# jianzhnie/ScaleRL

Measured on AMD Instinct MI355X. Metric: env_steps_per_sec, higher is better.
Workload: dtype bf16; 1 GPU; model=IMPALA AtariNet (3conv+FC512+2xLSTM519), algo=impala-vtrace, rollout_length=80, global_batch=256, seq_len=80, envs_per_actor=256, actors_per_rank=24, inference=gpu, parallelism=dp1

## Files before the change

scalerl_amd/ops/_backend.py:

```python

from __future__ import annotations

import ctypes
import os
import subprocess
import sys
from typing import Optional

import torch

_THIS_DIR = os.path.dirname(os.path.abspath(__file__))
_CSRC = os.path.join(_THIS_DIR, "csrc")
_SO_PATH = os.path.join(_THIS_DIR, "_hip_ops.so")

_LIB: Optional[ctypes.CDLL] = None
_LOAD_ERROR: Optional[str] = None


def hip_sources():
    return sorted(
        os.path.join(_CSRC, f) for f in os.listdir(_CSRC) if f.endswith(".hip"))


def build(verbose: bool = True, arch: str = "gfx950") -> str:
    srcs = hip_sources()
    hdrs = sorted(
        os.path.join(_CSRC, f) for f in os.listdir(_CSRC) if f.endswith(".h"))
    if os.path.exists(_SO_PATH):
        newest = max(os.path.getmtime(p) for p in srcs + hdrs)
        if os.path.getmtime(_SO_PATH) >= newest:
            return _SO_PATH
    hipcc = os.environ.get("HIPCC", "hipcc")
    cmd = [hipcc, f"--offload-arch={arch}", "-O3", "-std=c++17", "-shared",
           "-fPIC", "-lrocblas", "-o", _SO_PATH] + srcs
    if verbose:
        print("[scalerl_amd.ops] building:", " ".join(cmd), file=sys.stderr)
    subprocess.run(cmd, check=True)
    return _SO_PATH


_CONV_FWD = "bf16 bf16 f32? bf16 long int"
_CONV1_FWD_U8 = "u8 bf16 f32? bf16 long int"
_CONV_WGRAD = "bf16 bf16 f32 long long"
_CONV_WGRAD_V3 = "bf16 bf16 f32 long"
_CONV_DGRAD = "bf16 bf16 bf16 long"
_SIGNATURES = {
    "impala_fused_loss": "f32 f32 i64 f32 f32 f32 f32 float float float float"
                         " float long long long f32 f32 f32 f32?",
    "vtrace_from_log_rhos": "f32 f32 f32 f32 f32 float float float long long"
                            " f32 f32",
    "gae_scan": "f32 f32 f32 f32 float long long f32 f32",
    "discounted_returns": "f32 f32 f32? long long f32",
    "nstep_fold": "f32 f32 float long long long f32 f32 i32",
    "fused_rmsprop": "f32 f32 f32 f32? long float float float float float",
    "fused_adam": "f32 f32 f32 f32 long float float float float float long",
    "fused_polyak": "f32 f32 long float",
    "grad_clip_by_norm": "f32 long f32 float",
    "fused_td_loss": "f32 f32? f32 i64 f32 f32 f32? f32? f32? float long long"
                     " long int float long float float f32 f32 f32",
    "ppo_fused_loss": "f32 i64 f32 f32 f32 f32 float float float long long"
                      " f32 f32 f32",
    "per_update": "f32 long i64 f32 long",
    "per_sample": "f32 long long f32 long i64 f32",
    "per_leaf_min": "f32 long long i32",
    "lstm_mask_rows": "f32 f32 f32 f32 f32 long long",
    "lstm_cell_fwd": "f32 f32 f32 f32 f32? f32? f32? long long",
    "lstm_cell_bwd": "f32 f32 f32 f32 f32 f32? f32 f32 f32 long long",
    "masked_lstm_seq_fwd": "f32 f32 f32 f32 f32 f32 f32 f32 f32 long long long",
    "masked_lstm_seq_bwd": "f32 f32 f32 f32 f32 f32 f32 f32 f32 f32 long long"
                           " long",
    "frame_cast_u8_bf16": "u8 bf16 long",
    "mfma_selftest": "f32 f32 f32",
    "atari_encoder_fwd": "u8 bf16 f32 bf16 f32 bf16 f32 bf16? bf16? bf16 long",
    "atari_conv1_fwd_u8": _CONV1_FWD_U8,
    "atari_conv1_fwd_bf16": _CONV_FWD,
    "atari_conv2_fwd": _CONV_FWD,
    "atari_conv3_fwd": _CONV_FWD,
    "atari_conv2_fwd_v3": _CONV_FWD,
    "atari_conv3_fwd_v3": _CONV_FWD,
    "atari_conv1_wgrad_u8": "u8 bf16 f32 long long",
    "atari_conv2_wgrad": _CONV_WGRAD,
    "atari_conv3_wgrad": _CONV_WGRAD,
    "atari_conv1_wgrad_v3": "u8 bf16 f32 long",
    "atari_conv2_wgrad_v3": _CONV_WGRAD_V3,
    "atari_conv3_wgrad_v3": _CONV_WGRAD_V3,
    "atari_conv2_dgrad": _CONV_DGRAD,
    "atari_conv3_dgrad": _CONV_DGRAD,
    "atari_conv2_dgrad_v3": _CONV_DGRAD,
}

_DTYPES = {"f32": torch.float32, "i64": torch.int64, "i32": torch.int32,
           "bf16": torch.bfloat16, "u8": torch.uint8}
_SCALARS = {"long": ctypes.c_long, "int": ctypes.c_int,
            "float": ctypes.c_float}


class _Spec:
    __slots__ = ("words", "dtypes", "nullable", "argtypes", "fn")

    def __init__(self, words):
        self.words = words
        self.dtypes = tuple(_DTYPES.get(w.rstrip("?")) for w in words)
        self.nullable = tuple(w.endswith("?") for w in words)
        self.argtypes = [_SCALARS.get(w, ctypes.c_void_p) for w in words]
        self.argtypes.append(ctypes.c_void_p)
        self.fn = None


_SPECS = {name: _Spec(sig.split()) for name, sig in _SIGNATURES.items()}


def lib() -> ctypes.CDLL:
    global _LIB, _LOAD_ERROR
    if _LIB is not None:
        return _LIB
    if not os.path.exists(_SO_PATH):
        raise RuntimeError(
            f"scalerl_amd HIP kernel library not found at {_SO_PATH}. "
            f"Build it with `python -c 'from scalerl_amd.ops import _backend; "
            f"_backend.build()'` or `python setup.py build_ext --inplace`. "
            f"GPU execution without the native kernels is not supported.")
    try:
        loaded = ctypes.CDLL(_SO_PATH)
    except OSError as e:
        _LOAD_ERROR = str(e)
        raise RuntimeError(f"failed to load {_SO_PATH}: {e}") from e
    for name, spec in _SPECS.items():
        fn = getattr(loaded, name)
        fn.argtypes = spec.argtypes
        fn.restype = ctypes.c_int
        spec.fn = fn
    _LIB = loaded
    return _LIB


def available() -> bool:
    return os.path.exists(_SO_PATH)


def _reject(name: str, spec: _Spec, args) -> None:
    if len(args) != len(spec.words):
        raise TypeError(f"HIP kernel {name} takes {len(spec.words)} arguments "
                        f"({' '.join(spec.words)}), got {len(args)}")
    tensors = []
    for i, (a, dtype, nullable, word) in enumerate(
            zip(args, spec.dtypes, spec.nullable, spec.words)):
        where = f"HIP kernel {name}, argument {i} ({word})"
        if a is None:
            if nullable:
                continue
            raise TypeError(f"{where}: None given, the kernel takes " +
                            ("a number" if dtype is None
                             else "no null pointer") + " here")
        if dtype is None:
            continue
        if not isinstance(a, torch.Tensor):
            raise TypeError(f"{where}: expected a {dtype} tensor, got "
                            f"{type(a).__name__}")
        if a.dtype != dtype:
            raise TypeError(f"{where}: expected dtype {dtype}, got {a.dtype}")
        if not a.is_contiguous():
            raise ValueError(f"{where}: expected a contiguous tensor, got "
                             f"shape {tuple(a.shape)} stride {a.stride()}")
        tensors.append((where, a))
    for where, a in tensors:
        if not a.is_cuda:
            raise ValueError(f"{where}: expected a tensor on the current GPU, "
                             f"got device {a.device}")
    cur = torch.cuda.current_device()
    for where, a in tensors:
        if a.device.index != cur:
            raise ValueError(f"{where}: tensor is on {a.device} but the "
                             f"current device, whose stream the kernel is "
                             f"enqueued on, is cuda:{cur}")
    raise AssertionError(f"HIP kernel {name}: launch rejected valid arguments")


def launch(name: str, *args) -> None:
    spec = _SPECS.get(name)
    if spec is None:
        raise ValueError(f"unknown HIP kernel {name!r}")
    if len(args) != len(spec.words):
        _reject(name, spec, args)
    try:
        cur = torch.cuda.current_device()
    except (RuntimeError, AssertionError):
        cur = -2
    raw = []
    add = raw.append
    try:
        for a, dtype in zip(args, spec.dtypes):
            if dtype is None or a is None:
                add(a)
            elif (a.dtype is dtype and a.is_contiguous()
                  and a.get_device() == cur):
                add(a.data_ptr())
            else:
                _reject(name, spec, args)
    except AttributeError:
        _reject(name, spec, args)
    if None in raw and any(a is None and not ok
                           for a, ok in zip(args, spec.nullable)):
        _reject(name, spec, args)
    fn = spec.fn
    if fn is None:
        lib()
        fn = spec.fn
    ret = fn(*raw, torch._C._cuda_getCurrentRawStream(cur))
    if ret != 0:
        hint = ""
        if ret == -2:
            hint = " (action-space size exceeds kernel MAX_A)"
        elif ret == -3:
            hint = " (rollout length exceeds LDS budget)"
        elif ret == -4:
            hint = " (atom count outside the C51 kernel's 2..1024)"
        raise RuntimeError(
            f"HIP kernel {name} failed with code {ret}{hint}; "
            f"device={torch.cuda.get_device_name()}")
```

scalerl_amd/ops/csrc/lstm.hip:

```cpp

#include "lstm_cell.h"

extern "C" __global__ void lstm_mask_rows_kernel(
    const float* a, const float* b,
    const float* __restrict__ notdone,
    float* a_out, float* b_out, long B, long H) {
  const long total = B * H;
  for (long i = (long)blockIdx.x * blockDim.x + threadIdx.x; i < total;
       i += (long)gridDim.x * blockDim.x) {
    const float nd = notdone[i / H];
    a_out[i] = a[i] * nd;
    if (b != nullptr) b_out[i] = b[i] * nd;
  }
}

extern "C" __global__ void lstm_cell_fwd_kernel(
    float* __restrict__ gates,
    const float* __restrict__ c_in,
    float* __restrict__ h_out,
    float* __restrict__ c_out,
    const float* __restrict__ nd_next,
    float* __restrict__ h_in_next,
    float* __restrict__ c_in_next,
    long B, long H) {
  const long total = B * H;
  for (long i = (long)blockIdx.x * blockDim.x + threadIdx.x; i < total;
       i += (long)gridDim.x * blockDim.x) {
    const long b = i / H, j = i % H;
    float* grow = gates + b * 4 * H;
    const float ig = sigmoidf_(grow[j]);
    const float fg = sigmoidf_(grow[H + j]);
    const float gg = tanhf(grow[2 * H + j]);
    const float og = sigmoidf_(grow[3 * H + j]);
    const float c = fg * c_in[i] + ig * gg;
    const float h = og * tanhf(c);
    grow[j] = ig;
    grow[H + j] = fg;
    grow[2 * H + j] = gg;
    grow[3 * H + j] = og;
    c_out[i] = c;
    h_out[i] = h;
    if (nd_next != nullptr) {
      const float nd = nd_next[b];
      h_in_next[i] = h * nd;
      c_in_next[i] = c * nd;
    }
  }
}

extern "C" __global__ void lstm_cell_bwd_kernel(
    const float* __restrict__ gates,
    const float* __restrict__ c_in,
    const float* __restrict__ c_out,
    const float* __restrict__ d_hs_t,
    const float* __restrict__ g,
    const float* __restrict__ nd_next,
    const float* __restrict__ nd_t,
    float* dc_carry,
    float* __restrict__ dgates,
    long B, long H) {
  const long total = B * H;
  for (long i = (long)blockIdx.x * blockDim.x + threadIdx.x; i < total;
       i += (long)gridDim.x * blockDim.x) {
    const long b = i / H, j = i % H;
    const float* grow = gates + b * 4 * H;
    float* dgrow = dgates + b * 4 * H;
    const float ig = grow[j];
    const float fg = grow[H + j];
    const float gg = grow[2 * H + j];
    const float og = grow[3 * H + j];
    const float tc = tanhf(c_out[i]);
    const float gm = (nd_next != nullptr) ? g[i] * nd_next[b] : g[i];
    const float dh = d_hs_t[i] + gm;
    float tc2;
    {
#pragma clang fp contract(off)
      tc2 = tc * tc;
    }
    const float dc = dc_carry[i] + dh * og * (1.f - tc2);
    dgrow[j] = dc * gg * ig * (1.f - ig);
    dgrow[H + j] = dc * c_in[i] * fg * (1.f - fg);
    dgrow[2 * H + j] = dc * ig * (1.f - gg * gg);
    dgrow[3 * H + j] = dh * tc * og * (1.f - og);
    dc_carry[i] = (dc * fg) * nd_t[b];
  }
}

void lstm_launch_mask_rows(const float* a, const float* b, const float* notdone,
                           float* a_out, float* b_out, long B, long H,
                           hipStream_t stream) {
  hipLaunchKernelGGL(lstm_mask_rows_kernel,
                     dim3(grid_1d(B * H, LSTM_CELL_BLOCK)),
                     dim3(LSTM_CELL_BLOCK), 0, stream, a, b, notdone, a_out,
                     b_out, B, H);
}

void lstm_launch_cell_fwd(float* gates, const float* c_in, float* h_out,
                          float* c_out, const float* nd_next, float* h_in_next,
                          float* c_in_next, long B, long H,
                          hipStream_t stream) {
  hipLaunchKernelGGL(lstm_cell_fwd_kernel,
                     dim3(grid_1d(B * H, LSTM_CELL_BLOCK)),
                     dim3(LSTM_CELL_BLOCK), 0, stream, gates, c_in, h_out,
                     c_out, nd_next, h_in_next, c_in_next, B, H);
}

void lstm_launch_cell_bwd(const float* gates, const float* c_in,
                          const float* c_out, const float* d_hs_t,
                          const float* g, const float* nd_next,
                          const float* nd_t, float* dc_carry, float* dgates,
                          long B, long H, hipStream_t stream) {
  hipLaunchKernelGGL(lstm_cell_bwd_kernel,
                     dim3(grid_1d(B * H, LSTM_CELL_BLOCK)),
                     dim3(LSTM_CELL_BLOCK), 0, stream, gates, c_in, c_out,
                     d_hs_t, g, nd_next, nd_t, dc_carry, dgates, B, H);
}

extern "C" int lstm_mask_rows(const float* a, const float* b,
                              const float* notdone, float* a_out,
                              float* b_out, long B, long H,
                              hipStream_t stream) {
  if (B <= 0 || H <= 0) return 0;
  lstm_launch_mask_rows(a, b, notdone, a_out, b_out, B, H, stream);
  CHECK_LAUNCH();
  return 0;
}

extern "C" int lstm_cell_fwd(float* gates, const float* c_in, float* h_out,
                             float* c_out, const float* nd_next,
                             float* h_in_next, float* c_in_next, long B,
                             long H, hipStream_t stream) {
  if (B <= 0 || H <= 0) return 0;
  lstm_launch_cell_fwd(gates, c_in, h_out, c_out, nd_next, h_in_next,
                       c_in_next, B, H, stream);
  CHECK_LAUNCH();
  return 0;
}

extern "C" int lstm_cell_bwd(const float* gates, const float* c_in,
                             const float* c_out, const float* d_hs_t,
                             const float* g, const float* nd_next,
                             const float* nd_t, float* dc_carry,
                             float* dgates, long B, long H,
                             hipStream_t stream) {
  if (B <= 0 || H <= 0) return 0;
  lstm_launch_cell_bwd(gates, c_in, c_out, d_hs_t, g, nd_next, nd_t,
                       dc_carry, dgates, B, H, stream);
  CHECK_LAUNCH();
  return 0;
}
```

scalerl_amd/ops/csrc/lstm_cell.h:

```cpp
#pragma once

#include "common.h"

#define LSTM_CELL_BLOCK 256

void lstm_launch_mask_rows(const float* a, const float* b, const float* notdone,
                           float* a_out, float* b_out, long B, long H,
                           hipStream_t stream);

void lstm_launch_cell_fwd(float* gates, const float* c_in, float* h_out,
                          float* c_out, const float* nd_next, float* h_in_next,
                          float* c_in_next, long B, long H, hipStream_t stream);

void lstm_launch_cell_bwd(const float* gates, const float* c_in,
                          const float* c_out, const float* d_hs_t,
                          const float* g, const float* nd_next,
                          const float* nd_t, float* dc_carry, float* dgates,
                          long B, long H, hipStream_t stream);
```

scalerl_amd/ops/lstm.py:

```python

from __future__ import annotations

from typing import List, Tuple

import torch
import torch.nn as nn

from ._backend import launch


def _pointwise_fwd(gates: torch.Tensor, c_prev: torch.Tensor,
                   out_h: torch.Tensor = None, out_c: torch.Tensor = None):
    i, f, g, o = gates.chunk(4, dim=1)
    i, f, g, o = i.sigmoid(), f.sigmoid(), g.tanh(), o.sigmoid()
    c_new = f * c_prev + i * g
    h_new = o * torch.tanh(c_new)
    gates.copy_(torch.cat([i, f, g, o], dim=1))
    if out_h is not None:
        out_h.copy_(h_new)
        h_new = out_h
    if out_c is not None:
        out_c.copy_(c_new)
        c_new = out_c
    return h_new, c_new


def _pointwise_bwd(gates_act, c_prev, c_out, dh, dc_in,
                   out_dgates: torch.Tensor = None,
                   out_dc_prev: torch.Tensor = None):
    i, f, g, o = gates_act.chunk(4, dim=1)
    tc = torch.tanh(c_out)
    dc = dh * o * (1 - tc * tc)
    if dc_in is not None:
        dc = dc + dc_in
    di = dc * g * i * (1 - i)
    df = dc * c_prev * f * (1 - f)
    dg = dc * i * (1 - g * g)
    do = dh * tc * o * (1 - o)
    dgates = torch.cat([di, df, dg, do], dim=1)
    dc_prev = dc * f
    if out_dgates is not None:
        out_dgates.copy_(dgates)
        dgates = out_dgates
    if out_dc_prev is not None:
        out_dc_prev.copy_(dc_prev)
        dc_prev = out_dc_prev
    return dgates, dc_prev


def _grad_epilogue(dgates_all, x, hs_in, w_ih):
    T, B, I = x.shape
    dg2 = dgates_all.reshape(T * B, dgates_all.shape[-1])
    dx = (dg2 @ w_ih).view(T, B, I)
    dw_ih = dg2.t() @ x.reshape(T * B, I)
    dw_hh = dg2.t() @ hs_in.reshape(T * B, hs_in.shape[-1])
    db = dg2.sum(0)
    return dx, dw_ih, dw_hh, db


class _MaskedLSTMFn(torch.autograd.Function):

    @staticmethod
    @torch.amp.custom_fwd(device_type="cuda", cast_inputs=torch.float32)
    def forward(ctx, x, notdone, h0, c0, w_ih, w_hh, b_ih, b_hh):
        T, B, I = x.shape
        H = w_hh.shape[1]
        xg = torch.addmm(b_ih + b_hh, x.reshape(T * B, I), w_ih.t()).view(T, B, 4 * H)
        hs = torch.empty(T, B, H, device=x.device, dtype=x.dtype)
        cs_in = torch.empty(T, B, H, device=x.device, dtype=x.dtype)
        cs_out = torch.empty(T, B, H, device=x.device, dtype=x.dtype)
        hs_in = torch.empty(T, B, H, device=x.device, dtype=x.dtype)
        w_hh_t = w_hh.t()
        ctx.H = H
        if x.is_cuda:
            nd = notdone.reshape(T, B).contiguous()
            launch("lstm_mask_rows", h0.contiguous(), c0.contiguous(), nd[0],
                   hs_in[0], cs_in[0], B, H)
            for t in range(T):
                xg[t].addmm_(hs_in[t], w_hh_t)
                last = t == T - 1
                launch("lstm_cell_fwd",
                       xg[t], cs_in[t], hs[t], cs_out[t],
                       None if last else nd[t + 1],
                       None if last else hs_in[t + 1],
                       None if last else cs_in[t + 1], B, H)
            ctx.save_for_backward(x, nd, hs_in, cs_in, cs_out, xg, w_ih,
                                  w_hh)
            return hs, hs[T - 1].clone(), cs_out[T - 1].clone()
        h, c = h0.contiguous(), c0.contiguous()
        gates_all = torch.empty(T, B, 4 * H, device=x.device, dtype=x.dtype)
        for t in range(T):
            nd = notdone[t]
            h = torch.mul(h, nd, out=hs_in[t])
            c = torch.mul(c, nd, out=cs_in[t])
            torch.addmm(xg[t], h, w_hh_t, out=gates_all[t])
            h, c = _pointwise_fwd(gates_all[t], c, out_h=hs[t],
                                  out_c=cs_out[t])
        ctx.save_for_backward(x, notdone, hs_in, cs_in, cs_out, gates_all,
                              w_ih, w_hh)
        return hs, h.clone(), c.clone()

    @staticmethod
    @torch.amp.custom_bwd(device_type="cuda")
    def backward(ctx, d_hs, d_hT, d_cT):
        (x, notdone, hs_in, cs_in, cs_out, gates_all, w_ih,
         w_hh) = ctx.saved_tensors
        T, B, I = x.shape
        dgates_all = torch.empty_like(gates_all)
        if x.is_cuda:
            H = ctx.H
            nd = notdone
            d_hs_c = d_hs.contiguous()
            d_hT_c = d_hT.contiguous()
            dc_carry = d_cT.contiguous().clone()
            g = torch.empty_like(dc_carry)
            for t in range(T - 1, -1, -1):
                last = t == T - 1
                launch("lstm_cell_bwd",
                       gates_all[t], cs_in[t], cs_out[t],
                       d_hs_c[t], d_hT_c if last else g,
                       None if last else nd[t + 1], nd[t],
                       dc_carry, dgates_all[t], B, H)
                torch.mm(dgates_all[t], w_hh, out=g)
            dh0 = g.mul_(nd[0].unsqueeze(1))
            dx, dw_ih, dw_hh, db = _grad_epilogue(dgates_all, x, hs_in, w_ih)
            return dx, None, dh0, dc_carry, dw_ih, dw_hh, db, db
        dh_carry = d_hT.contiguous().clone()
        dc_carry = d_cT.contiguous().clone()
        dh_buf = torch.empty_like(dh_carry)
        dc_prev_buf = torch.empty_like(dc_carry)
        for t in range(T - 1, -1, -1):
            dh = torch.add(d_hs[t], dh_carry, out=dh_buf)
            dgates, dc_prev = _pointwise_bwd(
                gates_all[t], cs_in[t], cs_out[t], dh, dc_carry,
                out_dgates=dgates_all[t], out_dc_prev=dc_prev_buf)
            nd = notdone[t]
            torch.mm(dgates, w_hh, out=dh_carry)
            dh_carry.mul_(nd)
            torch.mul(dc_prev, nd, out=dc_carry)
        dx, dw_ih, dw_hh, db = _grad_epilogue(dgates_all, x, hs_in, w_ih)
        return dx, None, dh_carry, dc_carry, dw_ih, dw_hh, db, db


class _MaskedLSTMSeqFn(torch.autograd.Function):

    @staticmethod
    @torch.amp.custom_fwd(device_type="cuda", cast_inputs=torch.float32)
    def forward(ctx, x, notdone, h0, c0, w_ih, w_hh, b_ih, b_hh):
        T, B, I = x.shape
        H = w_hh.shape[1]
        dev = x.device
        xg = torch.addmm(b_ih + b_hh, x.reshape(T * B, I),
                         w_ih.t()).view(T, B, 4 * H).contiguous()
        hs = torch.empty(T, B, H, device=dev)
        hs_in = torch.empty(T, B, H, device=dev)
        cs_in = torch.empty(T, B, H, device=dev)
        cs_out = torch.empty(T, B, H, device=dev)
        nd = notdone.reshape(T, B).contiguous()
        w_hh_c = w_hh.contiguous()
        launch("masked_lstm_seq_fwd", xg, w_hh_c, nd, h0.contiguous(),
               c0.contiguous(), hs, hs_in, cs_in, cs_out, T, B, H)
        ctx.save_for_backward(x, nd, hs_in, cs_in, cs_out, xg, w_ih, w_hh_c)
        ctx.H = H
        return hs, hs[T - 1].clone(), cs_out[T - 1].clone()

    @staticmethod
    @torch.amp.custom_bwd(device_type="cuda")
    def backward(ctx, d_hs, d_hT, d_cT):
        x, nd, hs_in, cs_in, cs_out, gates_all, w_ih, w_hh = ctx.saved_tensors
        T, B, I = x.shape
        H = ctx.H
        dev = x.device
        dgates_all = torch.empty(T, B, 4 * H, device=dev)
        dh_carry = torch.empty(B, H, device=dev)
        dc_carry = d_cT.contiguous().clone()
        launch("masked_lstm_seq_bwd", gates_all, cs_in, cs_out,
               d_hs.contiguous(), d_hT.contiguous(), nd, w_hh, dgates_all,
               dh_carry, dc_carry, T, B, H)
        dx, dw_ih, dw_hh, db = _grad_epilogue(dgates_all, x, hs_in, w_ih)
        return dx, None, dh_carry, dc_carry, dw_ih, dw_hh, db, db


_USE_SEQ = None


def _use_seq_path() -> bool:
    global _USE_SEQ
    if _USE_SEQ is None:
        import os
        _USE_SEQ = os.environ.get("SCALERL_LSTM_SEQ", "1") != "0"
    return _USE_SEQ


class MaskedLSTM(nn.Module):

    def __init__(self, input_size: int, hidden_size: int, num_layers: int = 1):
        super().__init__()
        self.input_size, self.hidden_size = input_size, hidden_size
        self.num_layers = num_layers
        for k in range(num_layers):
            in_sz = input_size if k == 0 else hidden_size
            w_ih = nn.Parameter(torch.empty(4 * hidden_size, in_sz))
            w_hh = nn.Parameter(torch.empty(4 * hidden_size, hidden_size))
            b_ih = nn.Parameter(torch.empty(4 * hidden_size))
            b_hh = nn.Parameter(torch.empty(4 * hidden_size))
            for w in (w_ih, w_hh, b_ih, b_hh):
                nn.init.uniform_(w, -hidden_size ** -0.5, hidden_size ** -0.5)
            setattr(self, f"weight_ih_l{k}", w_ih)
            setattr(self, f"weight_hh_l{k}", w_hh)
            setattr(self, f"bias_ih_l{k}", b_ih)
            setattr(self, f"bias_hh_l{k}", b_hh)

    def initial_state(self, batch_size: int, device=None):
        z = torch.zeros(self.num_layers, batch_size, self.hidden_size,
                        device=device)
        return (z, z.clone())

    def forward(self, x: torch.Tensor, notdone: torch.Tensor,
                state: Tuple[torch.Tensor, torch.Tensor]):
        h0, c0 = state
        x = x.float()
        nd = notdone.unsqueeze(-1).float()
        hs_out: List[torch.Tensor] = []
        cs_out: List[torch.Tensor] = []
        out = x
        fn = (_MaskedLSTMSeqFn if (x.is_cuda and x.shape[0] > 1 and
                                   _use_seq_path())
              else _MaskedLSTMFn)
        for k in range(self.num_layers):
            out, hN, cN = fn.apply(
                out.contiguous(), nd, h0[k], c0[k],
                getattr(self, f"weight_ih_l{k}"),
                getattr(self, f"weight_hh_l{k}"),
                getattr(self, f"bias_ih_l{k}"),
                getattr(self, f"bias_hh_l{k}"))
            hs_out.append(hN)
            cs_out.append(cN)
        return out, (torch.stack(hs_out), torch.stack(cs_out))
```

scalerl_amd/parallel/inference.py:

```python

from __future__ import annotations

import queue
import time
from typing import Dict, List, Tuple

import torch


class InferenceSlots:

    def __init__(self, num_actors: int, envs_per_actor: int,
                 obs_shape: Tuple[int, ...], num_actions: int,
                 lstm_layers: int, lstm_hidden: int):
        A, E = num_actors, envs_per_actor
        self.num_actors, self.envs_per_actor = A, E
        self.num_actions = num_actions
        self.lstm_layers, self.lstm_hidden = lstm_layers, lstm_hidden

        def shared(shape, dtype):
            t = torch.zeros(shape, dtype=dtype)
            t.share_memory_()
            return t

        self.obs = shared((A, E, *obs_shape), torch.uint8)
        self.reward = shared((A, E), torch.float32)
        self.done = shared((A, E), torch.bool)
        self.last_action = shared((A, E), torch.int64)
        self.want_state = shared((A,), torch.int32)
        self.action = shared((A, E), torch.int64)
        self.logits = shared((A, E, num_actions), torch.float32)
        if lstm_hidden > 0:
            self.core_state = shared((A, 2, lstm_layers, E, lstm_hidden),
                                     torch.float32)
        else:
            self.core_state = None

    def tensors(self):
        ts = [self.obs, self.reward, self.done, self.last_action,
              self.want_state, self.action, self.logits]
        if self.core_state is not None:
            ts.append(self.core_state)
        return ts


class RemotePolicy:

    def __init__(self, actor_id: int, slots: InferenceSlots, req_q, sem):
        self.aid = actor_id
        self.slots = slots
        self.req_q = req_q
        self.sem = sem

    def request(self, obs, reward, done, last_action,
                want_state: bool = False) -> None:
        a = self.aid
        s = self.slots
        s.obs[a].copy_(obs)
        s.reward[a].copy_(reward)
        s.done[a].copy_(done)
        s.last_action[a].copy_(last_action)
        s.want_state[a] = 1 if want_state else 0
        self._want_state = want_state
        self.req_q.put(a)

    def wait(self):
        a = self.aid
        s = self.slots
        self.sem.acquire()
        state = s.core_state[a].clone() if (self._want_state and
                                            s.core_state is not None) else None
        return s.action[a].clone(), s.logits[a].clone(), state

    def __call__(self, obs, reward, done, last_action,
                 want_state: bool = False):
        self.request(obs, reward, done, last_action, want_state)
        return self.wait()


def inference_worker(device_index: int, model_kwargs: Dict, slots: InferenceSlots,
                     shared_flat: torch.Tensor, version: "mp.Value",
                     req_q, sems: List, stop_event, max_batch_actors: int = 0,
                     seed: int = 0, pause_flag=None, paused_ack=None,
                     as_thread: bool = False):
    from ..models.atari import AtariNet
    from .flat import FlatParams
    from .rollout import pin_tensor

    import os
    device = torch.device(f"cuda:{device_index}")
    if not as_thread:
        torch.manual_seed(seed)
        torch.cuda.set_device(device)
    stream = torch.cuda.Stream(device=device) if as_thread else None
    done_ev = torch.cuda.Event()
    model = AtariNet(**model_kwargs).to(device)
    model.train()
    flat = FlatParams(model, device=device)
    for t in slots.tensors():
        pin_tensor(t)
    if not as_thread:
        pin_tensor(shared_flat)
    inf_bf16 = os.environ.get("SCALERL_INF_BF16", "1") != "0"

    A, E = slots.num_actors, slots.envs_per_actor
    nact = slots.num_actions
    use_lstm = slots.core_state is not None
    if use_lstm:
        L, H = slots.lstm_layers, slots.lstm_hidden
        h_all = torch.zeros(L, A * E, H, device=device)
        c_all = torch.zeros(L, A * E, H, device=device)
    max_batch_actors = max_batch_actors or A
    seen_version = -1

    obs_d = torch.zeros((A, E, *slots.obs.shape[2:]), dtype=torch.uint8,
                        device=device)
    rew_d = torch.zeros((A, E), device=device)
    done_d = torch.zeros((A, E), dtype=torch.bool, device=device)
    lastact_d = torch.zeros((A, E), dtype=torch.int64, device=device)

    nonlocal_state = {"seen_version": seen_version}

    def run_round(ids):
        if version.value != nonlocal_state["seen_version"]:
            nonlocal_state["seen_version"] = version.value
            flat.load_from(shared_flat, non_blocking=False)

        for a in ids:
            obs_d[a].copy_(slots.obs[a], non_blocking=True)
            rew_d[a].copy_(slots.reward[a], non_blocking=True)
            done_d[a].copy_(slots.done[a], non_blocking=True)
            lastact_d[a].copy_(slots.last_action[a], non_blocking=True)
        inputs = {
            "obs": obs_d.reshape(1, A * E, *slots.obs.shape[2:]),
            "reward": rew_d.reshape(1, A * E),
            "done": done_d.reshape(1, A * E),
            "last_action": lastact_d.reshape(1, A * E),
        }
        state = ()
        snap = {}
        if use_lstm:
            for a in ids:
                if slots.want_state[a]:
                    snap[a] = (h_all[:, a * E:(a + 1) * E].clone(),
                               c_all[:, a * E:(a + 1) * E].clone())
            state = (h_all, c_all)
        if inf_bf16:
            with torch.autocast(device_type="cuda", dtype=torch.bfloat16):
                out, new_state = model(inputs, state)
        else:
            out, new_state = model(inputs, state)
        action = out["action"].view(A, E)
        logits = out["policy_logits"].view(A, E, nact)
        for a in ids:
            if use_lstm:
                sl = slice(a * E, (a + 1) * E)
                h_all[:, sl] = new_state[0][:, sl]
                c_all[:, sl] = new_state[1][:, sl]
            slots.action[a].copy_(action[a], non_blocking=True)
            slots.logits[a].copy_(logits[a], non_blocking=True)
            if a in snap:
                hj, cj = snap[a]
                slots.core_state[a][0].copy_(hj, non_blocking=True)
                slots.core_state[a][1].copy_(cj, non_blocking=True)
        done_ev.record(stream if stream is not None
                       else torch.cuda.current_stream(device))
        done_ev.synchronize()

    import contextlib
    with torch.no_grad():
        while not stop_event.is_set():
            if pause_flag is not None and pause_flag.value:
                torch.cuda.synchronize()
                if paused_ack is not None:
                    paused_ack.value = 1
                while pause_flag.value and not stop_event.is_set():
                    time.sleep(0.002)
                if paused_ack is not None:
                    paused_ack.value = 0
                continue
            try:
                first = req_q.get(timeout=0.2)
            except queue.Empty:
                continue
            if first is None:
                break
            ids = [first]
            while len(ids) < max_batch_actors:
                try:
                    nxt = req_q.get_nowait()
                except queue.Empty:
                    break
                if nxt is None:
                    stop_event.set()
                    break
                ids.append(nxt)
            sctx = (torch.cuda.stream(stream) if stream is not None
                    else contextlib.nullcontext())
            with sctx:
                run_round(ids)
            for a in ids:
                sems[a].release()
```

Before: 484,100 env-steps/s.

## Run inference only on requesting actors' rows with fused LSTM state gather/scatter kernels

Adds a compact inference path that packs only the actors in the current round into contiguous buffers instead of running the model over all A*E rows. New HIP kernels gather each actor's LSTM state with done-masking and snapshotting, then scatter the updated h/c back by actor id. The LSTM step is done manually with addmm plus a fused cell kernel. The path is on by default when the fused encoder and bf16 are in use. It adds warm-up rounds, refactors the worker into a class, and varies batch shapes per round, which may cost some kernel-selection or allocation overhead.

```diff
diff --git a/scalerl_amd/ops/_backend.py b/scalerl_amd/ops/_backend.py
--- a/scalerl_amd/ops/_backend.py
+++ b/scalerl_amd/ops/_backend.py
@@ -63,8 +63,9 @@
     "per_update": "f32 long i64 f32 long",
     "per_sample": "f32 long long f32 long i64 f32",
     "per_leaf_min": "f32 long long i32",
-    "lstm_mask_rows": "f32 f32 f32 f32 f32 long long",
-    "lstm_cell_fwd": "f32 f32 f32 f32 f32? f32? f32? long long",
+    "lstm_mask_rows": "f32 f32 f32? f32 f32 long long i32? i32? u8? f32? long"
+                      " long long",
+    "lstm_cell_fwd": "f32 f32 f32 f32 f32? f32? f32? long long i32? long long",
     "lstm_cell_bwd": "f32 f32 f32 f32 f32 f32? f32 f32 f32 long long",
     "masked_lstm_seq_fwd": "f32 f32 f32 f32 f32 f32 f32 f32 f32 long long long",
     "masked_lstm_seq_bwd": "f32 f32 f32 f32 f32 f32 f32 f32 f32 f32 long long"
diff --git a/scalerl_amd/ops/csrc/infer_step.hip b/scalerl_amd/ops/csrc/infer_step.hip
--- /dev/null
+++ b/scalerl_amd/ops/csrc/infer_step.hip
@@ -0,0 +1,81 @@
+
+#include "lstm_cell.h"
+
+#define INFER_BLOCK 256
+
+extern "C" __global__ void infer_state_gather_kernel(
+    const float* __restrict__ h_all,
+    const float* __restrict__ c_all,
+    const int* __restrict__ ids,
+    const int* __restrict__ want,
+    const unsigned char* __restrict__ done,
+    float* __restrict__ h_in,
+    float* __restrict__ c_in,
+    float* __restrict__ snap,
+    long n, long E, long R, long L, long H) {
+  const long M = n * E;
+  const long total = L * M * H;
+  const long A = R / E;
+  for (long i = (long)blockIdx.x * blockDim.x + threadIdx.x; i < total;
+       i += (long)gridDim.x * blockDim.x) {
+    const long k = i / (M * H), rem = i % (M * H);
+    const long r = rem / H, col = rem % H;
+    const long j = r / E, e = r % E;
+    const long a = ids[j];
+    if (a < 0 || a >= A) continue;
+    const long src = (k * R + a * E + e) * H + col;
+    const float h = h_all[src], c = c_all[src];
+    const float nd = done[r] ? 0.f : 1.f;
+    h_in[i] = h * nd;
+    c_in[i] = c * nd;
+    if (want[j]) {
+      const long dst = (((j * 2) * L + k) * E + e) * H + col;
+      snap[dst] = h;
+      snap[dst + L * E * H] = c;
+    }
+  }
+}
+
+extern "C" __global__ void infer_lstm_cell_kernel(
+    const float* __restrict__ gates,
+    const float* __restrict__ c_in,
+    const int* __restrict__ ids,
+    float* __restrict__ h_state,
+    float* __restrict__ c_state,
+    float* __restrict__ h_next,
+    long M, long E, long R, long H) {
+  const long total = M * H;
+  const long A = R / E;
+  for (long i = (long)blockIdx.x * blockDim.x + threadIdx.x; i < total;
+       i += (long)gridDim.x * blockDim.x) {
+    const long r = i / H, col = i % H;
+    const long a = ids[r / E];
+    const LstmCellStep s = lstm_cell_step(gates + r * 4 * H, H, col, c_in + i);
+    h_next[i] = s.h;
+    if (a < 0 || a >= A) continue;
+    const long dst = (a * E + r % E) * H + col;
+    h_state[dst] = s.h;
+    c_state[dst] = s.c;
+  }
+}
+
+void infer_launch_state_gather(const float* h_all, const float* c_all,
+                               const int* ids, const int* want,
+                               const unsigned char* done, float* h_in,
+                               float* c_in, float* snap, long n, long E,
+                               long R, long L, long H, hipStream_t stream) {
+  hipLaunchKernelGGL(infer_state_gather_kernel,
+                     dim3(grid_1d(L * n * E * H, INFER_BLOCK)),
+                     dim3(INFER_BLOCK), 0, stream, h_all, c_all, ids, want,
+                     done, h_in, c_in, snap, n, E, R, L, H);
+}
+
+void infer_launch_lstm_cell(const float* gates, const float* c_in,
+                            const int* ids, float* h_state, float* c_state,
+                            float* h_next, long M, long E, long R, long H,
+                            hipStream_t stream) {
+  hipLaunchKernelGGL(infer_lstm_cell_kernel,
+                     dim3(grid_1d(M * H, INFER_BLOCK)), dim3(INFER_BLOCK), 0,
+                     stream, gates, c_in, ids, h_state, c_state, h_next, M, E,
+                     R, H);
+}
diff --git a/scalerl_amd/ops/csrc/lstm.hip b/scalerl_amd/ops/csrc/lstm.hip
--- a/scalerl_amd/ops/csrc/lstm.hip
+++ b/scalerl_amd/ops/csrc/lstm.hip
@@ -28,16 +28,12 @@
        i += (long)gridDim.x * blockDim.x) {
     const long b = i / H, j = i % H;
     float* grow = gates + b * 4 * H;
-    const float ig = sigmoidf_(grow[j]);
-    const float fg = sigmoidf_(grow[H + j]);
-    const float gg = tanhf(grow[2 * H + j]);
-    const float og = sigmoidf_(grow[3 * H + j]);
-    const float c = fg * c_in[i] + ig * gg;
-    const float h = og * tanhf(c);
-    grow[j] = ig;
-    grow[H + j] = fg;
-    grow[2 * H + j] = gg;
-    grow[3 * H + j] = og;
+    const LstmCellStep s = lstm_cell_step(grow, H, j, c_in + i);
+    const float c = s.c, h = s.h;
+    grow[j] = s.ig;
+    grow[H + j] = s.fg;
+    grow[2 * H + j] = s.gg;
+    grow[3 * H + j] = s.og;
     c_out[i] = c;
     h_out[i] = h;
     if (nd_next != nullptr) {
@@ -118,8 +114,20 @@
 
 extern "C" int lstm_mask_rows(const float* a, const float* b,
                               const float* notdone, float* a_out,
-                              float* b_out, long B, long H,
-                              hipStream_t stream) {
+                              float* b_out, long B, long H, const int* ids,
+                              const int* want, const void* done, float* snap,
+                              long E, long R, long L, hipStream_t stream) {
+  if (ids != nullptr) {
+    if (want == nullptr || done == nullptr || snap == nullptr || b == nullptr ||
+        B < 0 || E < 1 || L < 1 || H < 1 || R < E || R % E != 0 || B > R / E)
+      return -1;
+    if (B == 0) return 0;
+    infer_launch_state_gather(a, b, ids, want, (const unsigned char*)done,
+                              a_out, b_out, snap, B, E, R, L, H, stream);
+    CHECK_LAUNCH();
+    return 0;
+  }
+  if (notdone == nullptr) return -1;
   if (B <= 0 || H <= 0) return 0;
   lstm_launch_mask_rows(a, b, notdone, a_out, b_out, B, H, stream);
   CHECK_LAUNCH();
@@ -129,7 +137,18 @@
 extern "C" int lstm_cell_fwd(float* gates, const float* c_in, float* h_out,
                              float* c_out, const float* nd_next,
                              float* h_in_next, float* c_in_next, long B,
-                             long H, hipStream_t stream) {
+                             long H, const int* ids, long E, long R,
+                             hipStream_t stream) {
+  if (ids != nullptr) {
+    if (nd_next != nullptr || c_in_next != nullptr || h_in_next == nullptr ||
+        B < 0 || E < 1 || H < 1 || B % E != 0 || R < E || R % E != 0 || B > R)
+      return -1;
+    if (B == 0) return 0;
+    infer_launch_lstm_cell(gates, c_in, ids, h_out, c_out, h_in_next, B, E, R,
+                           H, stream);
+    CHECK_LAUNCH();
+    return 0;
+  }
   if (B <= 0 || H <= 0) return 0;
   lstm_launch_cell_fwd(gates, c_in, h_out, c_out, nd_next, h_in_next,
                        c_in_next, B, H, stream);
diff --git a/scalerl_amd/ops/csrc/lstm_cell.h b/scalerl_amd/ops/csrc/lstm_cell.h
--- a/scalerl_amd/ops/csrc/lstm_cell.h
+++ b/scalerl_amd/ops/csrc/lstm_cell.h
@@ -3,6 +3,22 @@
 #include "common.h"
 
 #define LSTM_CELL_BLOCK 256
+
+struct LstmCellStep {
+  float ig, fg, gg, og, c, h;
+};
+
+__device__ __forceinline__ LstmCellStep lstm_cell_step(const float* grow,
+                                                       long H, long j,
+                                                       const float* c_in) {
+  const float ig = sigmoidf_(grow[j]);
+  const float fg = sigmoidf_(grow[H + j]);
+  const float gg = tanhf(grow[2 * H + j]);
+  const float og = sigmoidf_(grow[3 * H + j]);
+  const float c = fg * *c_in + ig * gg;
+  const float h = og * tanhf(c);
+  return {ig, fg, gg, og, c, h};
+}
 
 void lstm_launch_mask_rows(const float* a, const float* b, const float* notdone,
                            float* a_out, float* b_out, long B, long H,
@@ -17,3 +33,14 @@
                           const float* g, const float* nd_next,
                           const float* nd_t, float* dc_carry, float* dgates,
                           long B, long H, hipStream_t stream);
+
+void infer_launch_state_gather(const float* h_all, const float* c_all,
+                               const int* ids, const int* want,
+                               const unsigned char* done, float* h_in,
+                               float* c_in, float* snap, long n, long E,
+                               long R, long L, long H, hipStream_t stream);
+
+void infer_launch_lstm_cell(const float* gates, const float* c_in,
+                            const int* ids, float* h_state, float* c_state,
+                            float* h_next, long M, long E, long R, long H,
+                            hipStream_t stream);
diff --git a/scalerl_amd/ops/infer_step.py b/scalerl_amd/ops/infer_step.py
--- /dev/null
+++ b/scalerl_amd/ops/infer_step.py
@@ -0,0 +1,103 @@
+
+from __future__ import annotations
+
+from typing import List, Optional, Sequence, Tuple
+
+import torch
+import torch.nn.functional as F
+
+from ._backend import launch
+from .lstm import _pointwise_fwd
+
+
+def stage_ids(ids: Sequence[int], want: Sequence[int], num_actors: int,
+              device) -> Tuple[torch.Tensor, torch.Tensor]:
+    ids = [int(a) for a in ids]
+    if len(set(ids)) != len(ids) or any(a < 0 or a >= num_actors for a in ids):
+        raise ValueError(f"actor ids must be distinct and in "
+                         f"[0, {num_actors}): {ids}")
+    if len(want) != len(ids):
+        raise ValueError("one want flag per id")
+    return (torch.tensor(ids, dtype=torch.int32, device=device),
+            torch.tensor([int(bool(w)) for w in want], dtype=torch.int32,
+                         device=device))
+
+
+def core_input(feat: torch.Tensor, reward: torch.Tensor,
+               last_action: torch.Tensor, num_actions: int) -> torch.Tensor:
+    M = feat.shape[0]
+    one_hot = F.one_hot(last_action.view(M), num_actions).float()
+    clipped = torch.clamp(reward.view(M, 1), -1, 1)
+    return torch.cat([feat.float(), clipped, one_hot], dim=-1)
+
+
+def state_gather(h_all: torch.Tensor, c_all: torch.Tensor, ids: torch.Tensor,
+                 want: torch.Tensor, done: torch.Tensor, E: int):
+    L, R, H = h_all.shape
+    n = ids.shape[0]
+    M = n * E
+    dev = h_all.device
+    h_in = torch.empty(L, M, H, device=dev)
+    c_in = torch.empty(L, M, H, device=dev)
+    snap = torch.empty(n, 2, L, E, H, device=dev)
+    if h_all.is_cuda:
+        launch("lstm_mask_rows", h_all, c_all, None, h_in, c_in, n, H, ids,
+               want, done.reshape(M).view(torch.uint8), snap, E, R, L)
+        return h_in, c_in, snap
+    rows = (ids.long().view(n, 1) * E + torch.arange(E)).view(M)
+    nd = (~done.reshape(M)).float().view(1, M, 1)
+    h, c = h_all[:, rows], c_all[:, rows]
+    torch.mul(h, nd, out=h_in)
+    torch.mul(c, nd, out=c_in)
+    for j in range(n):
+        if int(want[j]):
+            snap[j, 0] = h[:, j * E:(j + 1) * E]
+            snap[j, 1] = c[:, j * E:(j + 1) * E]
+    return h_in, c_in, snap
+
+
+def lstm_cell(gates: torch.Tensor, c_in: torch.Tensor, ids: torch.Tensor,
+              h_state: torch.Tensor, c_state: torch.Tensor,
+              E: int) -> torch.Tensor:
+    M, H = c_in.shape
+    R = h_state.shape[0]
+    if gates.is_cuda:
+        h_next = torch.empty(M, H, device=gates.device)
+        launch("lstm_cell_fwd", gates, c_in, h_state, c_state, None, h_next,
+               None, M, H, ids, E, R)
+        return h_next
+    n = M // E
+    rows = (ids.long().view(n, 1) * E + torch.arange(E)).view(M)
+    h, c = _pointwise_fwd(gates.clone(), c_in)
+    h_state[rows] = h
+    c_state[rows] = c
+    return h
+
+
+def lstm_bias_sums(core) -> List[torch.Tensor]:
+    return [getattr(core, f"bias_ih_l{k}") + getattr(core, f"bias_hh_l{k}")
+            for k in range(core.num_layers)]
+
+
+@torch.no_grad()
+def policy_step(model, feat: torch.Tensor, reward: torch.Tensor,
+                done: torch.Tensor, last_action: torch.Tensor,
+                ids: torch.Tensor, want: torch.Tensor, h_all: torch.Tensor,
+                c_all: torch.Tensor, E: int,
+                generator: Optional[torch.Generator] = None,
+                bias: Optional[List[torch.Tensor]] = None):
+    core = model.core
+    if bias is None:
+        bias = lstm_bias_sums(core)
+    x = core_input(feat, reward, last_action, model.num_actions)
+    h_in, c_in, snap = state_gather(h_all, c_all, ids, want, done, E)
+    with torch.autocast(device_type=feat.device.type, enabled=False):
+        for k in range(core.num_layers):
+            gates = torch.addmm(bias[k], x,
+                                getattr(core, f"weight_ih_l{k}").t())
+            gates.addmm_(h_in[k], getattr(core, f"weight_hh_l{k}").t())
+            x = lstm_cell(gates, c_in[k], ids, h_all[k], c_all[k], E)
+        logits = F.linear(x, model.policy.weight, model.policy.bias)
+    action = torch.multinomial(F.softmax(logits, dim=-1), num_samples=1,
+                               generator=generator).squeeze(-1)
+    return action, logits, snap
diff --git a/scalerl_amd/ops/lstm.py b/scalerl_amd/ops/lstm.py
--- a/scalerl_amd/ops/lstm.py
+++ b/scalerl_amd/ops/lstm.py
@@ -75,7 +75,7 @@
         if x.is_cuda:
             nd = notdone.reshape(T, B).contiguous()
             launch("lstm_mask_rows", h0.contiguous(), c0.contiguous(), nd[0],
-                   hs_in[0], cs_in[0], B, H)
+                   hs_in[0], cs_in[0], B, H, None, None, None, None, 0, 0, 0)
             for t in range(T):
                 xg[t].addmm_(hs_in[t], w_hh_t)
                 last = t == T - 1
@@ -83,7 +83,7 @@
                        xg[t], cs_in[t], hs[t], cs_out[t],
                        None if last else nd[t + 1],
                        None if last else hs_in[t + 1],
-                       None if last else cs_in[t + 1], B, H)
+                       None if last else cs_in[t + 1], B, H, None, 0, 0)
             ctx.save_for_backward(x, nd, hs_in, cs_in, cs_out, xg, w_ih,
                                   w_hh)
             return hs, hs[T - 1].clone(), cs_out[T - 1].clone()
diff --git a/scalerl_amd/parallel/inference.py b/scalerl_amd/parallel/inference.py
--- a/scalerl_amd/parallel/inference.py
+++ b/scalerl_amd/parallel/inference.py
@@ -1,7 +1,9 @@
 
 from __future__ import annotations
 
+import os
 import queue
+import sys
 import time
 from typing import Dict, List, Tuple
 
@@ -78,59 +80,163 @@
         return self.wait()
 
 
-def inference_worker(device_index: int, model_kwargs: Dict, slots: InferenceSlots,
-                     shared_flat: torch.Tensor, version: "mp.Value",
-                     req_q, sems: List, stop_event, max_batch_actors: int = 0,
-                     seed: int = 0, pause_flag=None, paused_ack=None,
-                     as_thread: bool = False):
-    from ..models.atari import AtariNet
-    from .flat import FlatParams
-    from .rollout import pin_tensor
-
-    import os
-    device = torch.device(f"cuda:{device_index}")
-    if not as_thread:
-        torch.manual_seed(seed)
-        torch.cuda.set_device(device)
-    stream = torch.cuda.Stream(device=device) if as_thread else None
-    done_ev = torch.cuda.Event()
-    model = AtariNet(**model_kwargs).to(device)
-    model.train()
-    flat = FlatParams(model, device=device)
-    for t in slots.tensors():
-        pin_tensor(t)
-    if not as_thread:
-        pin_tensor(shared_flat)
-    inf_bf16 = os.environ.get("SCALERL_INF_BF16", "1") != "0"
-
-    A, E = slots.num_actors, slots.envs_per_actor
-    nact = slots.num_actions
-    use_lstm = slots.core_state is not None
-    if use_lstm:
-        L, H = slots.lstm_layers, slots.lstm_hidden
-        h_all = torch.zeros(L, A * E, H, device=device)
-        c_all = torch.zeros(L, A * E, H, device=device)
-    max_batch_actors = max_batch_actors or A
-    seen_version = -1
-
-    obs_d = torch.zeros((A, E, *slots.obs.shape[2:]), dtype=torch.uint8,
-                        device=device)
-    rew_d = torch.zeros((A, E), device=device)
-    done_d = torch.zeros((A, E), dtype=torch.bool, device=device)
-    lastact_d = torch.zeros((A, E), dtype=torch.int64, device=device)
-
-    nonlocal_state = {"seen_version": seen_version}
-
-    def run_round(ids):
-        if version.value != nonlocal_state["seen_version"]:
-            nonlocal_state["seen_version"] = version.value
-            flat.load_from(shared_flat, non_blocking=False)
+class InferenceRound:
+
+    _PHASES = ("copies_in", "enqueue", "copies_out", "event_wait")
+
+    def __init__(self, device, model_kwargs: Dict, slots: InferenceSlots,
+                 shared_flat: torch.Tensor, version, stream=None,
+                 pin_flat: bool = True):
+        from ..models import atari
+        from ..models.atari import AtariNet
+        from .flat import FlatParams
+        from .rollout import PinRegistry, pin_tensor
+
+        self.device = device
+        self.slots = slots
+        self.shared_flat = shared_flat
+        self.version = version
+        self.stream = stream
+        self.done_ev = torch.cuda.Event()
+        self.model = model = AtariNet(**model_kwargs).to(device)
+        model.train()
+        self.flat = FlatParams(model, device=device)
+        self.pins = PinRegistry()
+        for t in slots.tensors():
+            pin_tensor(t, self.pins)
+        if pin_flat:
+            pin_tensor(shared_flat, self.pins)
+        self.inf_bf16 = os.environ.get("SCALERL_INF_BF16", "1") != "0"
+
+        A, E = slots.num_actors, slots.envs_per_actor
+        self.A, self.E = A, E
+        self.use_lstm = slots.core_state is not None
+        if self.use_lstm:
+            L, H = slots.lstm_layers, slots.lstm_hidden
+            self.h_all = torch.zeros(L, A * E, H, device=device)
+            self.c_all = torch.zeros(L, A * E, H, device=device)
+        self.seen_version = -1
+
+        self.obs_d = torch.zeros((A, E, *slots.obs.shape[2:]),
+                                 dtype=torch.uint8, device=device)
+        self.rew_d = torch.zeros((A, E), device=device)
+        self.done_d = torch.zeros((A, E), dtype=torch.bool, device=device)
+        self.lastact_d = torch.zeros((A, E), dtype=torch.int64, device=device)
+
+        self.compact = (os.environ.get("SCALERL_INFER_COMPACT", "1") != "0"
+                        and device.type == "cuda" and self.inf_bf16
+                        and self.use_lstm and model.fused_encoder
+                        and atari.FUSED_ENCODER and not model.native_conv)
+        if self.compact:
+            self.idw_h = torch.zeros((2, A), dtype=torch.int32).pin_memory()
+            self.idw_np = self.idw_h.numpy()
+            self.idw_d = torch.zeros((2, A), dtype=torch.int32, device=device)
+            self.bias = None
+
+        self.stats = None
+        if os.environ.get("SCALERL_INFER_STATS", "0") == "1":
+            self.stats = {"rounds": 0, "hist": [0] * (A + 1), "t0": None,
+                          "t1": None, **{k: 0.0 for k in self._PHASES}}
+
+    def _tick(self, phase, t):
+        if self.stats is None:
+            return t
+        now = time.perf_counter()
+        self.stats[phase] += now - t
+        return now
+
+    def _refresh_weights(self):
+        if self.version.value != self.seen_version:
+            self.seen_version = self.version.value
+            self.flat.load_from(self.shared_flat, non_blocking=False)
+            if self.compact:
+                from ..ops import infer_step
+                self.bias = infer_step.lstm_bias_sums(self.model.core)
+
+    def _fence(self):
+        self.done_ev.record(self.stream if self.stream is not None
+                            else torch.cuda.current_stream(self.device))
+        self.done_ev.synchronize()
+
+    def run(self, ids, copy_out: bool = True):
+        st = self.stats
+        if st is not None:
+            st["rounds"] += 1
+            st["hist"][len(ids)] += 1
+            if st["t0"] is None:
+                st["t0"] = time.perf_counter()
+        if self.compact:
+            self._run_compact(ids, copy_out)
+        else:
+            self._run_all_rows(ids)
+        if st is not None:
+            st["t1"] = time.perf_counter()
+
+    def warm_up(self):
+        if not self.compact or self.stream is not None:
+            return
+        st, self.stats = self.stats, None
+        for n in range(1, self.A + 1):
+            self._run_compact(list(range(n)), copy_out=False)
+        self.h_all.zero_()
+        self.c_all.zero_()
+        self._fence()
+        self.stats = st
+
+    def _run_compact(self, ids, copy_out=True):
+        from ..ops import infer_step
+        slots, E = self.slots, self.E
+        n = len(ids)
+        assert len(set(ids)) == n and all(0 <= a < self.A for a in ids), ids
+        t = time.perf_counter() if self.stats is not None else 0.0
+        self._refresh_weights()
+        want = [int(slots.want_state[a]) for a in ids]
+        for j, a in enumerate(ids):
+            self.obs_d[j].copy_(slots.obs[a], non_blocking=True)
+            self.rew_d[j].copy_(slots.reward[a], non_blocking=True)
+            self.done_d[j].copy_(slots.done[a], non_blocking=True)
+            self.lastact_d[j].copy_(slots.last_action[a], non_blocking=True)
+            self.idw_np[0, j] = a
+            self.idw_np[1, j] = want[j]
+        self.idw_d.copy_(self.idw_h, non_blocking=True)
+        t = self._tick("copies_in", t)
+
+        M = n * E
+        with torch.autocast(device_type="cuda", dtype=torch.bfloat16):
+            feat = self.model.encode(
+                self.obs_d[:n].view(M, *slots.obs.shape[2:]))
+        action, logits, snap = infer_step.policy_step(
+            self.model, feat, self.rew_d[:n].view(M), self.done_d[:n].view(M),
+            self.lastact_d[:n].view(M), self.idw_d[0, :n], self.idw_d[1, :n],
+            self.h_all, self.c_all, E, bias=self.bias)
+        t = self._tick("enqueue", t)
+
+        if copy_out:
+            action = action.view(n, E)
+            logits = logits.view(n, E, slots.num_actions)
+            for j, a in enumerate(ids):
+                slots.action[a].copy_(action[j], non_blocking=True)
+                slots.logits[a].copy_(logits[j], non_blocking=True)
+                if want[j]:
+                    slots.core_state[a].copy_(snap[j], non_blocking=True)
+        t = self._tick("copies_out", t)
+        self._fence()
+        self._tick("event_wait", t)
+
+    def _run_all_rows(self, ids):
+        slots, A, E = self.slots, self.A, self.E
+        nact = slots.num_actions
+        obs_d, rew_d, done_d = self.obs_d, self.rew_d, self.done_d
+        lastact_d, model, use_lstm = self.lastact_d, self.model, self.use_lstm
+        t = time.perf_counter() if self.stats is not None else 0.0
+        self._refresh_weights()
 
         for a in ids:
             obs_d[a].copy_(slots.obs[a], non_blocking=True)
             rew_d[a].copy_(slots.reward[a], non_blocking=True)
             done_d[a].copy_(slots.done[a], non_blocking=True)
             lastact_d[a].copy_(slots.last_action[a], non_blocking=True)
+        t = self._tick("copies_in", t)
         inputs = {
             "obs": obs_d.reshape(1, A * E, *slots.obs.shape[2:]),
             "reward": rew_d.reshape(1, A * E),
@@ -140,16 +246,18 @@
         state = ()
         snap = {}
         if use_lstm:
+            h_all, c_all = self.h_all, self.c_all
             for a in ids:
                 if slots.want_state[a]:
                     snap[a] = (h_all[:, a * E:(a + 1) * E].clone(),
                                c_all[:, a * E:(a + 1) * E].clone())
             state = (h_all, c_all)
-        if inf_bf16:
+        if self.inf_bf16:
             with torch.autocast(device_type="cuda", dtype=torch.bfloat16):
                 out, new_state = model(inputs, state)
         else:
             out, new_state = model(inputs, state)
+        t = self._tick("enqueue", t)
         action = out["action"].view(A, E)
         logits = out["policy_logits"].view(A, E, nact)
         for a in ids:
@@ -163,12 +271,49 @@
                 hj, cj = snap[a]
                 slots.core_state[a][0].copy_(hj, non_blocking=True)
                 slots.core_state[a][1].copy_(cj, non_blocking=True)
-        done_ev.record(stream if stream is not None
-                       else torch.cuda.current_stream(device))
-        done_ev.synchronize()
+        t = self._tick("copies_out", t)
+        self._fence()
+        self._tick("event_wait", t)
+
+    def stats_report(self) -> str:
+        st = self.stats
+        if st is None or not st["rounds"]:
+            return ""
+        R = st["rounds"]
+        span = max(st["t1"] - st["t0"], 1e-9)
+        served = sum(n * c for n, c in enumerate(st["hist"]))
+        hist = " ".join(f"{n}:{c}" for n, c in enumerate(st["hist"]) if c)
+        split = "  ".join(f"{k} {1e6 * st[k] / R:.0f}" for k in self._PHASES)
+        return (f"[inference] path={'compact' if self.compact else 'all-rows'}"
+                f" rounds={R} rounds/s={R / span:.0f} "
+                f"mean actors/round={served / R:.2f} of {self.A}\n"
+                f"[inference] actors/round histogram: {hist}\n"
+                f"[inference] host us/round: {split}")
+
+
+def inference_worker(device_index: int, model_kwargs: Dict, slots: InferenceSlots,
+                     shared_flat: torch.Tensor, version: "mp.Value",
+                     req_q, sems: List, stop_event, max_batch_actors: int = 0,
+                     seed: int = 0, pause_flag=None, paused_ack=None,
+                     as_thread: bool = False):
+    device = torch.device(f"cuda:{device_index}")
+    if not as_thread:
+        torch.manual_seed(seed)
+        torch.cuda.set_device(device)
+    stream = torch.cuda.Stream(device=device) if as_thread else None
+    rnd = InferenceRound(device, model_kwargs, slots, shared_flat, version,
+                         stream=stream, pin_flat=not as_thread)
+    max_batch_actors = max_batch_actors or slots.num_actors
 
     import contextlib
+
+    def on_stream():
+        return (torch.cuda.stream(stream) if stream is not None
+                else contextlib.nullcontext())
+
     with torch.no_grad():
+        with on_stream():
+            rnd.warm_up()
         while not stop_event.is_set():
             if pause_flag is not None and pause_flag.value:
                 torch.cuda.synchronize()
@@ -195,9 +340,10 @@
                     stop_event.set()
                     break
                 ids.append(nxt)
-            sctx = (torch.cuda.stream(stream) if stream is not None
-                    else contextlib.nullcontext())
-            with sctx:
-                run_round(ids)
+            with on_stream():
+                rnd.run(ids)
             for a in ids:
                 sems[a].release()
+    report = rnd.stats_report()
+    if report:
+        print(report, file=sys.stderr, flush=True)
```

After: 534,000 env-steps/s, median of 6. 10.3% higher.
